# MoseleyBioinformaticsLab/pdb_eda

Measured on AMD Instinct MI355X. Metric: Mvoxels/s blob-labelled, higher is better.
Workload: dtype f32; 1 GPU; configs[1]: 256^3 synthetic CCP4 grid (gaussian-filtered noise, sigma_filter 1.5 voxels), fused green/red blob labelling at +-(mean+1.5*std), per-blob fp64 stats + dense int32 labels of both signs, map resident in HBM; labels=True, entries_per_rank=1

## Files before the change

### pdb_eda_amd/csrc/pdbeda_hip.hip

```cpp
#include <hip/hip_runtime.h>
#include <fcntl.h>
#include <sys/mman.h>
#include <sys/stat.h>
#include <unistd.h>
#include <cerrno>

#include <algorithm>
#include <chrono>
#include <thread>
#include <atomic>
#include <random>
#include <climits>
#include <cmath>
#include <cstdarg>
#include <cstdio>
#include <cstring>
#include <condition_variable>
#include <deque>
#include <map>
#include <mutex>
#include <string>
#include <vector>

#include "pdbeda_kernels.h"
// ... 1035 lines not shown
    pdbeda_ctx *ctx = m->ctx;
    HIP_TRY(ctx, hipSetDevice(ctx->device));
    return with_scratch(ctx, align_up(12 * n) + align_up(24 * n), [&](char *base) -> int {
        Carver cv(base);
        int32_t *d_crs = cv.take<int32_t>(3 * n);
        double *d_xyz = cv.take<double>(3 * n);
        const int32_t *in = pinned_in(ctx, crs, (size_t)(3 * n));
        if (!in) { HIP_TRY(ctx, h2d_one(ctx, d_crs, crs, (size_t)(12 * n))); in = d_crs; }
        double *res = pinned_out(ctx, xyz, (size_t)(3 * n));
        hipLaunchKernelGGL(k_crs2xyz, dim3(grid_for(n, 256)), dim3(256), 0, ctx->stream, m->geom_dev, in, n, res ? res : d_xyz);
        if (!res) HIP_TRY(ctx, d2h(ctx, xyz, d_xyz, 24 * n));
        return 0;
    });
}

extern "C" int pdbeda_xyz2crs(pdbeda_map *m, const double *xyz, int64_t n, int32_t *crs) {
    if (!m || (n > 0 && (!crs || !xyz)) || n < 0) return PDBEDA_ERR_ARGUMENT;
    if (n == 0) return PDBEDA_OK;
    pdbeda_ctx *ctx = m->ctx;
    HIP_TRY(ctx, hipSetDevice(ctx->device));
    return with_scratch(ctx, align_up(12 * n) + align_up(24 * n), [&](char *base) -> int {
        Carver cv(base);
        double *d_xyz = cv.take<double>(3 * n);
        int32_t *d_crs = cv.take<int32_t>(3 * n);
        const double *in = pinned_in(ctx, xyz, (size_t)(3 * n));
        if (!in) { HIP_TRY(ctx, h2d_one(ctx, d_xyz, xyz, (size_t)(24 * n))); in = d_xyz; }
        int32_t *res = pinned_out(ctx, crs, (size_t)(3 * n));
        hipLaunchKernelGGL(k_xyz2crs, dim3(grid_for(n, 256)), dim3(256), 0, ctx->stream, m->geom_dev, in, n, res ? res : d_crs);
        if (!res) HIP_TRY(ctx, d2h(ctx, crs, d_crs, 12 * n));
        return 0;
    });
}

static size_t job_carve(Job &job, char *base, int n_vols, int64_t total_words, int64_t total_keys, int64_t max_runs,
                        int64_t max_blobs, size_t extra_labels, int32_t **labels_out, int64_t n_tiles = 0, int64_t max_comps = -1) {
    if (max_comps < 0) max_comps = max_runs;
    job.run_cap = (uint32_t)max_runs; job.comp_cap = (uint32_t)max_comps; job.blob_cap = (uint32_t)std::min<int64_t>(max_blobs, 0xffffffffll);
    Carver cv(base);
    job.n_vols = n_vols;
    job.total_words = total_words;
    job.key_words = (total_keys + 63) / 64;
    job.n_fine = (int32_t)((job.key_words + KEY_FINE - 1) / KEY_FINE);
    job.fine_shift = 4;
    while (((int64_t)KEY_GROUPS << job.fine_shift) < job.n_fine) job.fine_shift++;
    job.fine_per_group = 1 << job.fine_shift;
    job.n_groups = (job.n_fine + job.fine_per_group - 1) / job.fine_per_group;
    job.vols = cv.take<VolDesc>(std::max(n_vols, 1));
    job.ctr = cv.take<Counters>(1);
    job.mask = cv.take<uint64_t>(total_words);
    job.key_bits = cv.take<uint64_t>((size_t)(job.key_words + KEY_FINE - 1) / KEY_FINE * KEY_FINE);
    job.n_fine_alloc = (int32_t)((job.n_fine + job.fine_per_group - 1) / job.fine_per_group * job.fine_per_group);
    job.fine_count = cv.take<uint32_t>((size_t)std::max(job.n_fine_alloc / 2, 8));
    job.mid_count = cv.take<uint32_t>((size_t)(job.key_words + KEY_FINE - 1) / KEY_FINE * (KEY_FINE / 16));
    job.group_count = (n_tiles && job.fine_shift > 4) ? cv.take<uint32_t>(KEY_GROUPS) : nullptr;
    job.run_base = cv.take<uint32_t>(total_words);
    job.comps_are_runs = n_tiles ? 0 : 1;
    job.comp_of_run = n_tiles ? cv.take<uint32_t>(max_runs) : nullptr;
    job.label_of_comp = n_tiles ? cv.take<int32_t>(max_comps) : nullptr;
    job.word_comps = n_tiles ? cv.take<uint8_t>((size_t)n_tiles * 2 * 256 * 8) : nullptr;
    job.unit_done = n_tiles ? cv.take<uint32_t>((size_t)n_tiles) : nullptr;
    job.unit_flag = n_tiles ? cv.take<uint32_t>(4) : nullptr;
    job.tile_mode = n_tiles ? cv.take<uint8_t>(n_tiles) : nullptr;
    job.tile_runs = n_tiles ? cv.take<uint32_t>(n_tiles) : nullptr;
    job.root_mask = n_tiles ? cv.take<uint64_t>((size_t)n_tiles * 4) : nullptr;
    job.n_tiles = (int32_t)n_tiles;
    if (n_tiles) {
        const int64_t nt = n_tiles, nfc = job.n_fine_alloc / 2, nmid = (job.key_words + KEY_FINE - 1) / KEY_FINE * (KEY_FINE / 16);
        job.clear_bits = (int32_t)((job.key_words + nt - 1) / nt);
        job.clear_fine = (int32_t)((nfc + nt - 1) / nt);
        job.clear_mid = (int32_t)((nmid + nt - 1) / nt);
    }
    job.inbox = n_tiles ? cv.take<InboxEntry>((size_t)n_tiles * INBOX_CAP) : nullptr;
    job.inbox_count = n_tiles ? cv.take<uint32_t>((size_t)n_tiles * INBOX_STRIDE) : nullptr;
    job.vol_sign[0] = job.vol_sign[1] = 1;
    job.parent = cv.take<int32_t>(max_comps);
    job.kpar = n_tiles ? cv.take<unsigned long long>(max_comps) : nullptr;
    job.r_n = cv.take<uint32_t>(max_comps);
    job.r_sum = cv.take<long long>((size_t)7 * max_comps);
    job.r_sum_stride = max_comps;
    job.r_c = cv.take<long long>(max_comps);
    job.r_r = cv.take<long long>(max_comps);
    job.r_s = cv.take<long long>(max_comps);
    job.r_key = cv.take<unsigned long long>(max_comps);
    job.r_rank = cv.take<uint32_t>(max_comps);
    job.b_n = cv.take<int64_t>(max_blobs);
    job.b_key = cv.take<int64_t>(max_blobs);
    job.b_total = cv.take<double>(max_blobs);
    job.b_centroid = cv.take<double>(3 * max_blobs);
    job.b_center = cv.take<double>(3 * max_blobs);
    job.b_volume = cv.take<double>(max_blobs);
    job.b_group = cv.take<int32_t>(max_blobs);
    int32_t *lab = extra_labels ? cv.take<int32_t>(extra_labels) : nullptr;
    if (labels_out) *labels_out = lab;
    return cv.off;
}

static int engine_enqueue(pdbeda_ctx *ctx, pdbeda_map *m, Job &job, int64_t max_runs, bool labelled = false, bool unordered = false) {
    hipStream_t st = ctx->stream;
    const unsigned run_grid = grid_for(max_runs, 256, 2048);
    if (job.total_words > 0 && !labelled) {
        {
            PROF(ctx, "k_run_index");
            static const int force_wpb = [] { const char *e = getenv("PDBEDA_RUNINDEX_WPB"); return e ? atoi(e) : 0; }();
            if (force_wpb != 256 && (force_wpb == 64 || (job.total_words < 256ll * 2048 && job.total_words > 64ll * job.n_vols))) hipLaunchKernelGGL(k_run_index<64>, dim3(grid_for(job.total_words, 64, 1ll << 30)), dim3(256), 0, st, job, m->dens, m->geom_dev);
            else hipLaunchKernelGGL(k_run_index<256>, dim3(grid_for(job.total_words, 256, 1ll << 30)), dim3(256), 0, st, job, m->dens, m->geom_dev);
        }
        { PROF(ctx, "k_union"); hipLaunchKernelGGL(k_union, dim3(grid_for(job.total_words * 4, 256, 1ll << 30)), dim3(256), 0, st, job); }
// ... 79 lines not shown
    const int64_t worst_unit = (int64_t)((uc + 1) / 2) * ur * us * n_planes + 1;
    if (tile_runs + worst_unit >= (1ll << 31))
        return fail(ctx, PDBEDA_ERR_ARGUMENT, "grid too large for whole-map labelling: %d x %d x %d voxels need %lld run ids (limit 2^31: about 1100^3 for a fused job)",
                    uc, ur, us, (long long)(tile_runs + worst_unit));
    const int64_t unit_ids = tier == 0 ? std::min<int64_t>(worst_unit, std::max<int64_t>(65536, tile_runs / 4)) : worst_unit;
    const int64_t max_blobs = tier == 0 ? std::min<int64_t>(worst_blobs, std::max<int64_t>(4096, total_keys / 32)) : worst_blobs;
    const int64_t max_runs = tile_runs + unit_ids, max_comps = tile_comps + unit_ids;

    int rc_fix = map_fix_mul(m);
    if (rc_fix) return rc_fix;
    Job job;
    memset(&job, 0, sizeof job);
    job.fix_mul = m->fix_mul;
    size_t need = job_carve(job, nullptr, n_planes, total_words, total_keys, max_runs, max_blobs, lab_elems, nullptr, tiles_pp, max_comps);
    Arena arena;
    int rc = arena_get(ctx, need, &arena);
    if (rc) return rc;
    int32_t *labels_dev = nullptr;
    job_carve(job, arena.base, n_planes, total_words, total_keys, max_runs, max_blobs, lab_elems, &labels_dev, tiles_pp, max_comps);
    job.vol_sign[0] = td.sign[0];
    job.vol_sign[1] = td.sign[1];
    job.unit_form = unit_form;
    static std::atomic<uint32_t> g_epoch{[] {
        uint32_t seed;
        try { seed = (uint32_t)std::random_device{}(); }
        catch (...) { seed = (uint32_t)std::chrono::steady_clock::now().time_since_epoch().count() ^ ((uint32_t)getpid() * 2654435761u); }
        return seed | 1u;
    }()};
    do { job.epoch = g_epoch.fetch_add(1u); } while (job.epoch == 0u || job.epoch == 0xffffffffu);

    JobInit init;
    memset(&init, 0, sizeof init);
    for (int p = 0; p < n_planes; ++p) {
        VolDesc &v = init.v[p];
        v.dim[0] = uc; v.dim[1] = ur; v.dim[2] = us;
        v.org[0] = v.org[1] = v.org[2] = 0;
        v.row_words = row_words;
        v.group = p;
        v.word_base = words_pp * p;
        v.key_base = keys_pp * p;
    }
    init.runs0 = (unsigned)tile_runs;
    init.comps0 = (unsigned)tile_comps;
    hipStream_t st = ctx->stream;
    int pair_slots = PAIR_SLOTS;
    if (ctx->debug_edge_cap > 0) { pair_slots = 1; while (pair_slots * 2 <= std::min<int64_t>(ctx->debug_edge_cap, PAIR_SLOTS)) pair_slots *= 2; }
    switch (td.cw) {
        case 1: launch_tile_label<1>(ctx, (unsigned)tiles_pp, job, m->dens, m->geom_dev, td, init, pair_slots); break;
        case 2: launch_tile_label<2>(ctx, (unsigned)tiles_pp, job, m->dens, m->geom_dev, td, init, pair_slots); break;
        case 3: launch_tile_label<3>(ctx, (unsigned)tiles_pp, job, m->dens, m->geom_dev, td, init, pair_slots); break;
        default: launch_tile_label<4>(ctx, (unsigned)tiles_pp, job, m->dens, m->geom_dev, td, init, pair_slots); break;
    }
    { PROF(ctx, "k_resolve_tiles"); hipLaunchKernelGGL(k_resolve_tiles, dim3((unsigned)tiles_pp + 64u), dim3(256), 0, st, job, (int)tiles_pp); }
    if (job.group_count) { PROF(ctx, "k_group_counts"); hipLaunchKernelGGL(k_group_counts, dim3((unsigned)(job.n_groups + 255) / 256u), dim3(256), 0, st, job); }
    if (labels) {
        PROF(ctx, "k_labels_tiles");
        launch_labels<true>(ctx, job, td, labels_dev, m->geom_dev);
    } else {
        PROF(ctx, "k_emit_tiles");
        hipLaunchKernelGGL(k_emit_tiles, dim3(std::min<unsigned>(512u, ((unsigned)tiles_pp + 1u) / 2u)), dim3(256), 0, st, job, m->geom_dev);
    }
    hipError_t e = hipGetLastError();
    if (e != hipSuccess) { arena_put(ctx, arena); return fail(ctx, PDBEDA_ERR_DEVICE, "whole-map labelling launch: %s", hipGetErrorString(e)); }
    out->job = job; out->arena = arena; out->td = td; out->labels_dev = labels_dev; out->labels = labels; out->bytes = need;
    return PDBEDA_OK;
}

static int full_blobs_impl(pdbeda_map *m, float cut_pos, float cut_neg, bool want_pos, bool want_neg, uint32_t flags,
                           pdbeda_bloblist **out_pos, pdbeda_bloblist **out_neg) {
    pdbeda_ctx *ctx = m->ctx;
    WholeMapJob wj;
    const int tier = ctx->debug_worst_case_arena ? 1 : 0, form = tier;
    int rc = whole_map_enqueue(m, cut_pos, cut_neg, want_pos, want_neg, flags, tier, form, &wj);
    if (rc) return rc;
    const int n_planes = (want_pos ? 1 : 0) + (want_neg ? 1 : 0);
    pdbeda_bloblist *first = nullptr;
    for (int p = 0; p < n_planes; ++p) {
        pdbeda_bloblist *bl = new_list(ctx, m);
        bl->job = wj.job;
        bl->td = wj.td;
        bl->vol_lo = p;
        bl->vol_hi = p + 1;
        bl->whole_map = true;
        bl->sign = wj.td.sign[p];
        if (p == 0) { bl->arena = wj.arena; bl->owns_arena = true; first = bl; }
        else { bl->owns_arena = false; bl->sibling = first; first->sibling = bl; }
        bl->labels_dev = wj.labels_dev;
        bl->labels_done = wj.labels;
        bl->cut_pos = cut_pos; bl->cut_neg = cut_neg; bl->want_pos = want_pos; bl->want_neg = want_neg; bl->flags = flags; bl->tier = tier; bl->unit_form = form;
        bl->job_bytes = wj.bytes;
        if (bl->sign > 0) *out_pos = bl; else *out_neg = bl;
    }
    return PDBEDA_OK;
}

extern "C" int pdbeda_full_blobs(pdbeda_map *m, float cutoff, uint32_t flags, pdbeda_bloblist **out) {
    if (!m || !out) return PDBEDA_ERR_ARGUMENT;
    *out = nullptr;
    if (cutoff == 0.0f || cutoff != cutoff) return fail(m->ctx, PDBEDA_ERR_ARGUMENT, "cutoff must be non-zero (the reference returns None)");
    pdbeda_bloblist *dummy = nullptr;
    if (cutoff > 0) return full_blobs_impl(m, cutoff, 0.0f, true, false, flags, out, &dummy);
    return full_blobs_impl(m, 0.0f, cutoff, false, true, flags, &dummy, out);
}

extern "C" int pdbeda_full_blobs_pm(pdbeda_map *m, float cutoff_pos, float cutoff_neg, uint32_t flags, pdbeda_bloblist **green,
                                    pdbeda_bloblist **red) {
    if (!m || !green || !red) return PDBEDA_ERR_ARGUMENT;
// ... 1779 lines not shown
```

### pdb_eda_amd/csrc/pdbeda_kernels.h

```cpp
#pragma once
#include "pdbeda_device.h"

namespace pdbeda {

struct VolDesc {
    int32_t dim[3];
    int32_t org[3];
    int32_t row_words;
    int32_t group;
    int64_t word_base;
    int64_t key_base;
};

struct FixSums {
    long long rho, c_lo, c_hi, r_lo, r_hi, s_lo, s_hi;
};
__device__ inline long long fix_of(double v, double mul) { return __double2ll_rn(v * mul); }
__device__ inline void fix_limbs(__int128 v, long long &lo, long long &hi) {
    lo = (long long)(unsigned long long)((unsigned __int128)v & 0xffffffffu);
    hi = (long long)(v >> 32);
}
__device__ inline double fix_moment(long long lo, long long hi) { return (double)hi * 4294967296.0 + (double)lo; }
__device__ inline FixSums fix_sums(long long F, long long m_c, long long m_r, long long m_s, long long c0, long long r0, long long s0) {
    FixSums o;
// ... 531 lines not shown
    unsigned long long c = 0, r = 0, sv = 0, key = ~0ull;
    if (root >= 0) {
        n = job.r_n[i]; sum = fix_load(job, i);
        c = (unsigned long long)job.r_c[i]; r = (unsigned long long)job.r_r[i]; sv = (unsigned long long)job.r_s[i]; key = job.r_key[i];
    }
    unsigned long long todo = __ballot(root >= 0);
    while (todo) {
        const int first = ctz64(todo);
        const int r0 = __shfl(root, first);
        const bool mine = root == r0;
        const unsigned long long group = __ballot(mine);
        todo &= ~group;
        uint32_t gn = mine ? n : 0u;
        FixSums g_sum = mine ? sum : fix_zero();
        unsigned long long g_c = mine ? c : 0ull, g_r = mine ? r : 0ull, g_s = mine ? sv : 0ull, g_key = mine ? key : ~0ull;
        if (group & (group - 1)) {
#pragma unroll
            for (int d = 32; d > 0; d >>= 1) {
                gn += __shfl_xor(gn, d);
                g_sum.rho += __shfl_xor(g_sum.rho, d);
                g_sum.c_lo += __shfl_xor(g_sum.c_lo, d); g_sum.c_hi += __shfl_xor(g_sum.c_hi, d);
                g_sum.r_lo += __shfl_xor(g_sum.r_lo, d); g_sum.r_hi += __shfl_xor(g_sum.r_hi, d);
                g_sum.s_lo += __shfl_xor(g_sum.s_lo, d); g_sum.s_hi += __shfl_xor(g_sum.s_hi, d);
                g_c += __shfl_xor(g_c, d); g_r += __shfl_xor(g_r, d); g_s += __shfl_xor(g_s, d);
                const unsigned long long k2 = __shfl_xor(g_key, d);
                g_key = k2 < g_key ? k2 : g_key;
            }
        }
        if (lane == first) {
            atomicAdd(&job.r_n[r0], gn);
            fix_fold(job, (uint32_t)r0, g_sum);
            atomicAdd((unsigned long long *)&job.r_c[r0], g_c);
            atomicAdd((unsigned long long *)&job.r_r[r0], g_r);
            atomicAdd((unsigned long long *)&job.r_s[r0], g_s);
            atomicMin(&job.r_key[r0], g_key);
        }
    }
}
__global__ void __launch_bounds__(256) k_resolve(Job job, int slots) {
    const uint32_t n_runs = n_components(job);
    const int lane = lane_id();
    const uint32_t stride = gridDim.x * blockDim.x;
    for (uint32_t i0 = blockIdx.x * blockDim.x + (threadIdx.x & ~63u); i0 < n_runs; i0 += stride)
        resolve_wave(job, i0 + (uint32_t)lane, i0 + (uint32_t)lane < n_runs, lane, slots != 0);
}

template <typename JobRef>
__device__ __forceinline__ void paint_key(const JobRef &job, unsigned long long key) {
    const uint32_t f = (uint32_t)((key >> 6) / KEY_FINE);
    const uint32_t cell = (uint32_t)(key >> 8);
    atomicOr((unsigned long long *)&job.key_bits[key >> 6], 1ull << (key & 63));
    atomicAdd(&job.mid_count[cell >> 2], 1u << ((cell & 3u) * 8u));
    atomicAdd(&job.fine_count[f >> 1], 1u << ((f & 1u) * 16u));
}

__global__ void __launch_bounds__(256) k_paint_keys(Job job) {
    const uint32_t n_runs = n_components(job);
    for (uint32_t i = blockIdx.x * blockDim.x + threadIdx.x; i < n_runs; i += gridDim.x * blockDim.x) {
        const int32_t par = job.parent[i];
        const uint32_t cnt = job.r_n[i];
        const unsigned long long key = job.r_key[i];
        if (par != (int32_t)i || cnt == 0u) continue;
        paint_key(job, key);
    }
}

template <int CTRL, int ROW_MASK = 0xf>
__device__ __forceinline__ uint32_t dpp0(uint32_t x) {
    return (uint32_t)__builtin_amdgcn_update_dpp(0, (int)x, CTRL, ROW_MASK, 0xf, true);
}
constexpr int DPP_ROW_SHR = 0x110, DPP_WAVE_SHR1 = 0x138, DPP_ROW_BCAST15 = 0x142, DPP_ROW_BCAST31 = 0x143;
__device__ __forceinline__ uint32_t half_scan(uint32_t x) {
    x += dpp0<DPP_ROW_SHR + 1>(x);
    x += dpp0<DPP_ROW_SHR + 2>(x);
    x += dpp0<DPP_ROW_SHR + 4>(x);
    x += dpp0<DPP_ROW_SHR + 8>(x);
    x += dpp0<DPP_ROW_BCAST15, 0xa>(x);
    return x;
}

__device__ __forceinline__ uint32_t wave_scan(uint32_t x) {
    x = half_scan(x);
    x += dpp0<DPP_ROW_BCAST31, 0xc>(x);
    return x;
}
__device__ __forceinline__ uint32_t sum_u16x8(const uint4 q) {
    const uint32_t a = (q.x & 0xffffu) + (q.x >> 16), b = (q.y & 0xffffu) + (q.y >> 16), c = (q.z & 0xffffu) + (q.z >> 16), d = (q.w & 0xffffu) + (q.w >> 16);
    return (a + b) + (c + d);
}
__device__ __forceinline__ uint32_t sum_u16_first(const uint4 q, int take) {
    const uint32_t w[4] = {q.x, q.y, q.z, q.w};
    uint32_t acc = 0;
#pragma unroll
    for (int k = 0; k < 4; ++k) acc += (2 * k < take ? (w[k] & 0xffffu) : 0u) + (2 * k + 1 < take ? (w[k] >> 16) : 0u);
    return acc;
}

template <int NT>
struct RankTableLoads {
    static constexpr int PER = KEY_GROUPS / NT;
    uint4 q[2 * PER];
    uint32_t v[PER];
    bool summed;
};
template <int NT = 256, typename JobRef = Job>
__device__ __forceinline__ void rank_table_issue(const JobRef &job, RankTableLoads<NT> &ld) {
    constexpr int PER = KEY_GROUPS / NT;
    const int tid = threadIdx.x;
    const int G = job.fine_per_group, n_groups = job.n_groups, Q = G / 8;
    const uint4 *fine4 = reinterpret_cast<const uint4 *>(job.fine_count);
    ld.summed = Q != 2;
    if (Q == 2) {
#pragma unroll
        for (int k = 0; k < PER; ++k) {
            const int e = tid * PER + k;
            ld.q[2 * k] = e < n_groups ? fine4[(size_t)e * 2] : make_uint4(0, 0, 0, 0);
            ld.q[2 * k + 1] = e < n_groups ? fine4[(size_t)e * 2 + 1] : make_uint4(0, 0, 0, 0);
        }
    } else if (job.group_count) {
        const uint32_t *gc = job.group_count;
#pragma unroll
        for (int k = 0; k < PER; ++k) {
            const int e = tid * PER + k;
            ld.v[k] = e < n_groups ? gc[e] : 0u;
        }
    } else {
#pragma unroll
        for (int k = 0; k < PER; ++k) {
            const int e = tid * PER + k;
            uint32_t acc = 0;
            if (e < n_groups)
                for (int j = 0; j < Q; ++j) acc += sum_u16x8(fine4[(size_t)e * Q + j]);
            ld.v[k] = acc;
        }
    }
}
template <int NT = 256>
__device__ __forceinline__ uint32_t rank_table_finish(RankTableLoads<NT> &ld, uint32_t *s_pre , uint32_t *s_wave ) {
    constexpr int PER = KEY_GROUPS / NT;
    const int tid = threadIdx.x, lane = tid & 63, wv = tid >> 6;
    if (!ld.summed) {
#pragma unroll
        for (int k = 0; k < PER; ++k) ld.v[k] = sum_u16x8(ld.q[2 * k]) + sum_u16x8(ld.q[2 * k + 1]);
    }
    uint32_t mine = 0;
#pragma unroll
    for (int k = 0; k < PER; ++k) mine += ld.v[k];
    const uint32_t x = wave_scan(mine);
    if (lane == 63) s_wave[wv] = x;
    __syncthreads();
    uint32_t pre = x - mine, total = 0;
#pragma unroll
    for (int k = 0; k < NT / 64; ++k) { const uint32_t w = s_wave[k]; pre += k < wv ? w : 0u; total += w; }
#pragma unroll
    for (int k = 0; k < PER; ++k) { s_pre[tid * PER + k] = pre; pre += ld.v[k]; }
    __syncthreads();
    return total;
}
template <int NT = 256, typename JobRef = Job>
__device__ inline uint32_t rank_table_lds(const JobRef &job, uint32_t *s_pre , uint32_t *s_wave ) {
    RankTableLoads<NT> ld;
    rank_table_issue<NT>(job, ld);
    return rank_table_finish<NT>(ld, s_pre, s_wave);
}

__global__ void __launch_bounds__(256) k_group_counts(Job job) {
    const int e = (int)(blockIdx.x * blockDim.x + threadIdx.x);
    if (e >= job.n_groups) return;
    const int Q = job.fine_per_group / 8;
    const uint4 *fine4 = reinterpret_cast<const uint4 *>(job.fine_count) + (size_t)e * Q;
    uint32_t acc = 0;
    for (int j = 0; j < Q; j += 4) {
        const uint4 a = fine4[j], b = fine4[j + 1], c = fine4[j + 2], d = fine4[j + 3];
        acc += (sum_u16x8(a) + sum_u16x8(b)) + (sum_u16x8(c) + sum_u16x8(d));
    }
    job.group_count[e] = acc;
}

struct RankLoads {
    uint4 q0, q1;
    uint2 mid;
    ulonglong2 b0, b1;
};
template <typename JobRef>
__device__ __forceinline__ void rank_issue(const JobRef &job, unsigned long long key, RankLoads &ld) {
    const uint32_t kw = (uint32_t)(key >> 6), f = kw / (uint32_t)KEY_FINE, e = f >> 4;
    const uint4 *fine4 = reinterpret_cast<const uint4 *>(job.fine_count) + (size_t)e * 2;
    ld.q0 = fine4[0]; ld.q1 = fine4[1];
    ld.mid = reinterpret_cast<const uint2 *>(job.mid_count)[f];
    const ulonglong2 *bits2 = reinterpret_cast<const ulonglong2 *>(job.key_bits + (kw & ~3u));
    ld.b0 = bits2[0]; ld.b1 = bits2[1];
}
__device__ __forceinline__ uint32_t rank_finish(const uint32_t *s_pre, unsigned long long key, const RankLoads &ld) {
    const uint32_t kw = (uint32_t)(key >> 6), f = kw / (uint32_t)KEY_FINE, e = f >> 4;
    const int nf = (int)(f & 15u), cell = (int)((kw & (uint32_t)(KEY_FINE - 1)) >> 2), wi = (int)(kw & 3u);
    uint32_t rank = s_pre[e] + sum_u16_first(ld.q0, nf) + sum_u16_first(ld.q1, nf - 8);
    const uint32_t lo = cell >= 4 ? ld.mid.x : (ld.mid.x & ((1u << (8 * cell)) - 1u));
    const uint32_t hi = cell > 4 ? (ld.mid.y & ((1u << (8 * (cell - 4))) - 1u)) : 0u;
    rank += __builtin_amdgcn_sad_u8(lo, 0u, 0u) + __builtin_amdgcn_sad_u8(hi, 0u, 0u);
    const uint64_t below = bits_below((int)(key & 63));
    const uint64_t w[4] = {ld.b0.x, ld.b0.y, ld.b1.x, ld.b1.y};
#pragma unroll
    for (int k = 0; k < 4; ++k) rank += (uint32_t)popc64(k < wi ? w[k] : (k == wi ? w[k] & below : 0ull));
    return rank;
}
template <typename JobRef>
__device__ inline uint32_t rank_of_key(const JobRef &job, const uint32_t *s_pre, unsigned long long key) {
    const int shift = job.fine_shift;
    if (shift == 4) {
        RankLoads ld;
        rank_issue(job, key, ld);
        return rank_finish(s_pre, key, ld);
    }
    const uint32_t kw = (uint32_t)(key >> 6), f = kw / (uint32_t)KEY_FINE, e = f >> shift;
    const int Q = 1 << (shift - 3);
    uint32_t rank = s_pre[e];
    const uint4 *fine4 = reinterpret_cast<const uint4 *>(job.fine_count) + (size_t)e * Q;
    const int nf = (int)(f - (e << shift));
    const uint2 mid = reinterpret_cast<const uint2 *>(job.mid_count)[f];
    const ulonglong2 *bits2 = reinterpret_cast<const ulonglong2 *>(job.key_bits + (kw & ~3u));
    const int cell = (int)((kw & (uint32_t)(KEY_FINE - 1)) >> 2);
    const int wi = (int)(kw & 3u);
    const ulonglong2 b0 = bits2[0], b1 = bits2[1];
    for (int k = 0; k * 8 < nf; ++k) rank += sum_u16_first(fine4[k], nf - k * 8);
    {
        const uint32_t lo = cell >= 4 ? mid.x : (mid.x & ((1u << (8 * cell)) - 1u));
        const uint32_t hi = cell > 4 ? (mid.y & ((1u << (8 * (cell - 4))) - 1u)) : 0u;
        rank += __builtin_amdgcn_sad_u8(lo, 0u, 0u) + __builtin_amdgcn_sad_u8(hi, 0u, 0u);
    }
    const uint64_t below = bits_below((int)(key & 63));
    const uint64_t w[4] = {b0.x, b0.y, b1.x, b1.y};
#pragma unroll
    for (int k = 0; k < 4; ++k) rank += (uint32_t)popc64(k < wi ? w[k] : (k == wi ? w[k] & below : 0ull));
    return rank;
}

__device__ __forceinline__ int nth_set_bit(uint64_t m, int k) {
    int pos = 0;
#pragma unroll
    for (int w = 32; w > 0; w >>= 1) {
        const int c = popc64(m & ((1ull << w) - 1ull));
        if (k >= c) { k -= c; m >>= w; pos += w; }
    }
    return pos;
}

template <typename JobRef>
__device__ __forceinline__ void emit_row_ranked(const JobRef &job, const Geom &g, bool whole_map, int64_t key_base1, uint32_t id, uint32_t n_vox,
                                                unsigned long long first_key, const FixSums &fs, long long ic, long long ir, long long is, uint32_t rank) {
    const double tot_q = (double)fs.rho, rc = fix_moment(fs.c_lo, fs.c_hi), rr = fix_moment(fs.r_lo, fs.r_hi), rs = fix_moment(fs.s_lo, fs.s_hi);
    const double tot = tot_q / job.fix_mul;
    const int vi = whole_map ? ((int64_t)first_key >= key_base1 ? 1 : 0) : find_vol_by_key(job.vols, job.n_vols, (int64_t)first_key);
    if (whole_map) job.label_of_comp[id] = job.vol_sign[vi] > 0 ? 1 + (int32_t)rank : -1 - (int32_t)rank;
    const VolDesc vd = job.vols[vi];
    job.r_rank[id] = rank;
    if (rank >= job.blob_cap) return;
    const double n = (double)n_vox;
    double wc[3] = {rc / tot_q, rr / tot_q, rs / tot_q};
    double cc[3] = {(double)ic / n, (double)ir / n, (double)is / n};
    double xyz[3];
    crs2xyz_frac(g, wc, xyz);
    job.b_centroid[3 * rank + 0] = xyz[0];
    job.b_centroid[3 * rank + 1] = xyz[1];
    job.b_centroid[3 * rank + 2] = xyz[2];
    crs2xyz_frac(g, cc, xyz);
    job.b_center[3 * rank + 0] = xyz[0];
    job.b_center[3 * rank + 1] = xyz[1];
    job.b_center[3 * rank + 2] = xyz[2];
    job.b_n[rank] = (int64_t)n_vox;
    job.b_total[rank] = tot;
    job.b_volume[rank] = g.unit_volume * n;
    job.b_key[rank] = (int64_t)first_key - vd.key_base;
    job.b_group[rank] = vd.group;
}
template <typename JobRef>
__device__ __forceinline__ void emit_row(const JobRef &job, const Geom &g, const uint32_t *s_pre, bool whole_map, int64_t key_base1, uint32_t id,
                                         uint32_t n_vox, unsigned long long first_key, const FixSums &fs, long long ic, long long ir, long long is) {
    emit_row_ranked(job, g, whole_map, key_base1, id, n_vox, first_key, fs, ic, ir, is, rank_of_key(job, s_pre, first_key));
}

template <typename JobRef>
__device__ inline void emit_ids(const JobRef &job, const Geom &g, const uint32_t *s_pre, bool whole_map, int64_t key_base1, uint32_t first, uint32_t n_comp,
                                uint32_t block, uint32_t n_blocks) {
    const uint32_t stride = n_blocks * blockDim.x;
    uint32_t i = first + block * blockDim.x + threadIdx.x;
    int32_t par = i < n_comp ? job.parent[i] : -1;
    uint32_t cnt = i < n_comp ? job.r_n[i] : 0u;
    unsigned long long key = i < n_comp ? job.r_key[i] : 0ull;
    for (; i < n_comp; i += stride) {
        const bool root = par == (int32_t)i && cnt != 0u;
        const uint32_t nx = i + stride;
        const int32_t par_next = nx < n_comp ? job.parent[nx] : -1;
        const uint32_t cnt_next = nx < n_comp ? job.r_n[nx] : 0u;
        const unsigned long long key_next = nx < n_comp ? job.r_key[nx] : 0ull;
        if (root) emit_row(job, g, s_pre, whole_map, key_base1, i, cnt, key, fix_load(job, i), job.r_c[i], job.r_r[i], job.r_s[i]);
        par = par_next;
        cnt = cnt_next;
        key = key_next;
    }
}

__global__ void __launch_bounds__(256) k_emit(Job job, const Geom *__restrict__ gp) {
    __shared__ uint32_t s_pre[KEY_GROUPS];
    __shared__ uint32_t s_wave[4];
    const uint32_t total = rank_table_lds(job, s_pre, s_wave);
    emit_ids(job, *gp, s_pre, false, INT64_MAX, 0u, n_components(job), blockIdx.x, gridDim.x);
    if (blockIdx.x == 0 && threadIdx.x == 0) {
        job.ctr->n_blobs = total;
        job.ctr->n_blobs_vol0 = total;
        if (total > job.blob_cap) atomicOr(&job.ctr->overflow, 2u);
    }
}

__global__ void __launch_bounds__(256) k_emit_tiles(Job job, const Geom *__restrict__ gp) {
    __shared__ uint32_t s_pre[KEY_GROUPS];
    __shared__ uint32_t s_wave[4];
    __shared__ unsigned long long s_acc[2][10][TILE_COMPS];
    __shared__ uint32_t s_accn[2][TILE_COMPS];
    const int half = threadIdx.x >> 7, k0 = threadIdx.x & 127;
    const int n_tiles = job.n_tiles;
    int tile = (int)blockIdx.x * 2 + half;
    uint64_t rm[4] = {0ull, 0ull, 0ull, 0ull};
    uint32_t n_in = 0;
    if (tile < n_tiles) {
#pragma unroll
        for (int q = 0; q < 4; ++q) rm[q] = job.root_mask[(size_t)tile * 4 + q];
        n_in = job.inbox_count[(size_t)tile * INBOX_STRIDE];
    }
    const int64_t key_base1 = job.n_vols > 1 ? job.vols[1].key_base : INT64_MAX;
    const uint32_t total = rank_table_lds(job, s_pre, s_wave);
    const Geom &g = *gp;
    for (int t0 = (int)blockIdx.x * 2; t0 < n_tiles; t0 += (int)gridDim.x * 2) {
        tile = t0 + half;
        n_in = min(n_in, (uint32_t)INBOX_CAP);
        const int next = tile + (int)gridDim.x * 2;
        uint64_t nm[4] = {0ull, 0ull, 0ull, 0ull};
        uint32_t n_in_next = 0;
        if (next < n_tiles) {
#pragma unroll
            for (int q = 0; q < 4; ++q) nm[q] = job.root_mask[(size_t)next * 4 + q];
            n_in_next = job.inbox_count[(size_t)next * INBOX_STRIDE];
        }
        InboxEntry e0, e1;
        const bool have0 = (uint32_t)k0 < n_in, have1 = (uint32_t)k0 + 128u < n_in;
        if (have0) e0 = job.inbox[(size_t)tile * INBOX_CAP + k0];
        if (have1) e1 = job.inbox[(size_t)tile * INBOX_CAP + k0 + 128];
        if (n_in != 0u) {
#pragma unroll
            for (int f = 0; f < 10; ++f) { s_acc[half][f][k0] = 0ull; s_acc[half][f][k0 + 128] = 0ull; }
            s_accn[half][k0] = 0u; s_accn[half][k0 + 128] = 0u;
        }
        __syncthreads();
        auto absorb = [&](const InboxEntry &e) {
            const uint32_t l = e.local;
            atomicAdd(&s_accn[half][l], e.n);
            atomicAdd(&s_acc[half][0][l], (unsigned long long)e.sum.rho);
            atomicAdd(&s_acc[half][1][l], (unsigned long long)e.sum.c_lo); atomicAdd(&s_acc[half][2][l], (unsigned long long)e.sum.c_hi);
            atomicAdd(&s_acc[half][3][l], (unsigned long long)e.sum.r_lo); atomicAdd(&s_acc[half][4][l], (unsigned long long)e.sum.r_hi);
            atomicAdd(&s_acc[half][5][l], (unsigned long long)e.sum.s_lo); atomicAdd(&s_acc[half][6][l], (unsigned long long)e.sum.s_hi);
            atomicAdd(&s_acc[half][7][l], e.c); atomicAdd(&s_acc[half][8][l], e.r); atomicAdd(&s_acc[half][9][l], e.s);
        };
        if (have0) absorb(e0);
        if (have1) absorb(e1);
        __syncthreads();
        const int c0 = popc64(rm[0]), c1 = c0 + popc64(rm[1]), c2 = c1 + popc64(rm[2]), n_roots = c2 + popc64(rm[3]);
        for (int k = k0; k < n_roots; k += 128) {
            const int q = k < c0 ? 0 : (k < c1 ? 1 : (k < c2 ? 2 : 3));
            const int before = q == 0 ? 0 : (q == 1 ? c0 : (q == 2 ? c1 : c2));
            const uint64_t word = q == 0 ? rm[0] : (q == 1 ? rm[1] : (q == 2 ? rm[2] : rm[3]));
            const uint32_t l = (uint32_t)(64 * q + nth_set_bit(word, k - before));
            const uint32_t id = (uint32_t)tile * (uint32_t)TILE_COMPS + l;
            uint32_t n_vox = job.r_n[id];
            const unsigned long long key = job.r_key[id];
            FixSums fs = fix_load(job, id);
            long long ic = job.r_c[id], ir = job.r_r[id], is = job.r_s[id];
            if (n_in != 0u) {
                n_vox += s_accn[half][l];
                fs.rho += (long long)s_acc[half][0][l];
                fs.c_lo += (long long)s_acc[half][1][l]; fs.c_hi += (long long)s_acc[half][2][l];
                fs.r_lo += (long long)s_acc[half][3][l]; fs.r_hi += (long long)s_acc[half][4][l];
                fs.s_lo += (long long)s_acc[half][5][l]; fs.s_hi += (long long)s_acc[half][6][l];
                ic += (long long)s_acc[half][7][l]; ir += (long long)s_acc[half][8][l]; is += (long long)s_acc[half][9][l];
            }
// ... 1281 lines not shown
```

### pdb_eda_amd/csrc/pdbeda_tile.h

```cpp
#pragma once
#include "pdbeda_kernels.h"
#include <type_traits>

namespace pdbeda {

constexpr int TILE_R = 8, TILE_S = 8;
constexpr int RCAP = 1408;
constexpr int RCAP_DENSE = 4096;
constexpr int CCAP = 256;
static_assert(CCAP == TILE_COMPS, "k_emit walks the tiles' component ranges");
constexpr int VCAP = 3584;
constexpr int FACE_K = 7;

struct TileDims {
    int cw;
    int ctiles, rtiles, stiles;
    int n_planes;
    int uc, ur, us, row_words;
    int nc, nr;
    float cut[2];
    int sign[2];
};

__host__ __device__ inline int64_t tile_index(const TileDims &td, int plane, int wq, int r, int s) {
// ... 632 lines not shown
    const unsigned long long *comps64 = reinterpret_cast<const unsigned long long *>(lj.word_comps);
    auto word_at = [&](int q, int r, int s, int wq) { return (int64_t)q * plane_words + ((int64_t)s * ur + r) * row_words + wq; };
    auto comps_at = [&](uint32_t tl, int q, int r, int s, int wl) { return ((size_t)tl * 2 + q) * 256 + ((s & 7) * TILE_R + (r & 7)) * CW + wl; };
    auto comp_by_run = [&](int64_t w, uint32_t k) { return lj.comp_of_run[lj.run_base[w] + k]; };

    const int fq = tid / (FACE_PAIRS * 4), frem = tid % (FACE_PAIRS * 4), ft = frem >> 2, fwl = frem & 3;
    int rl = 0, sl = 0, dr = 0, ds = -1;
    bool task = tid < 2 * FACE_PAIRS * 4 && fq < td.n_planes && fwl < CW && w0 + fwl < row_words;
    if (ft < 8) { rl = 0; sl = ft; dr = -1; ds = 0; }
    else if (ft < 16) { rl = 0; sl = ft - 8; dr = -1; }
    else if (ft < 23) { rl = ft - 15; sl = 0; dr = -1; }
    else if (ft < 31) { rl = ft - 23; sl = 0; dr = 0; }
    else if (ft < 39) { rl = ft - 31; sl = 0; dr = 1; }
    else { rl = 7; sl = ft - 38; dr = 1; }
    const int r = rt * TILE_R + rl, s = st * TILE_S + sl, r2 = r + dr, s2 = s + ds;
    if (r >= ur || s >= us || r2 < 0 || r2 >= ur || s2 < 0) task = false;
    const uint32_t tile_b = task ? (uint32_t)(((s2 >> 3) * td.rtiles + (r2 >> 3)) * td.ctiles + ct) : 0u;
    const int64_t wA = task ? word_at(fq, r, s, w0 + fwl) : 0, wB = task ? word_at(fq, r2, s2, w0 + fwl) : 0;
    uint64_t mA = 0ull, mB = 0ull;
    unsigned long long cA = 0ull, cB = 0ull;
    uint32_t modes = 0u;
    if (task) {
        mA = lj.mask[wA]; mB = lj.mask[wB];
        cA = comps64[comps_at((uint32_t)tile, fq, r, s, fwl)]; cB = comps64[comps_at(tile_b, fq, r2, s2, fwl)];
        modes = (uint32_t)lj.tile_mode[tile] | (uint32_t)lj.tile_mode[tile_b];
    }
    uint32_t tiles5[5];
    {
        const int drs[5] = {0, -1, -1, 0, 1}, dss[5] = {0, 0, -1, -1, -1};
#pragma unroll
        for (int j = 0; j < 5; ++j) {
            const int r5 = rt + drs[j], s5 = st + dss[j];
            tiles5[j] = (r5 >= 0 && r5 < td.rtiles && s5 >= 0) ? (uint32_t)((s5 * td.rtiles + r5) * td.ctiles + ct) : 0xffffffffu;
        }
    }
    constexpr int KPL = (5 * KPH + NTH - 1) / NTH;
    kp_t kp_pre[KPL];
#pragma unroll
    for (int k = 0; k < KPL; ++k) {
        const int e = tid + k * NTH, j = e / KPH;
        const uint32_t t5 = j == 0 ? tiles5[0] : (j == 1 ? tiles5[1] : (j == 2 ? tiles5[2] : (j == 3 ? tiles5[3] : tiles5[4])));
        kp_pre[k] = (e < 5 * KPH && t5 != 0xffffffffu) ? kuf_load(lj.kpar, t5 * (uint32_t)CCAP + (uint32_t)(e % KPH)) : KP_UNUSED;
    }
    {
        const int64_t key_words = lj.key_words;
        const int64_t lo = (int64_t)lj.clear_bits * tile, hi = lo + lj.clear_bits < key_words ? lo + lj.clear_bits : key_words;
        for (int64_t i = lo + tid; i < hi; i += NTH) lj.key_bits[i] = 0ull;
        const int64_t nfc = lj.n_fine_alloc / 2;
        const int64_t clo = (int64_t)lj.clear_fine * tile, chi = clo + lj.clear_fine < nfc ? clo + lj.clear_fine : nfc;
        for (int64_t i = clo + tid; i < chi; i += NTH) lj.fine_count[i] = 0u;
        const int64_t nmid = (key_words + KEY_FINE - 1) / KEY_FINE * (KEY_FINE / 16);
        const int64_t mlo = (int64_t)lj.clear_mid * tile, mhi = mlo + lj.clear_mid < nmid ? mlo + lj.clear_mid : nmid;
        for (int64_t i = mlo + tid; i < mhi; i += NTH) lj.mid_count[i] = 0u;
        if (tid == 0) lj.inbox_count[(size_t)tile * INBOX_STRIDE] = 0u;
    }
    for (int i = tid; i < pair_slots; i += NTH) s_set[i] = 0ull;
#pragma unroll
    for (int k = 0; k < KPL; ++k) {
        const int e = tid + k * NTH;
        if (e < 5 * KPH) (&s_kp[0][0])[e] = kp_pre[k];
    }
    lds_barrier();
    auto val_of = [&](uint32_t id) -> kp_t {
        const uint32_t t = id / (uint32_t)CCAP;
#pragma unroll
        for (int j = 0; j < 5; ++j)
            if (t == tiles5[j] && (id % (uint32_t)CCAP) < (uint32_t)KPH) return s_kp[j][id % (uint32_t)CCAP];
        return kuf_load(lj.kpar, id);
    };
    const uint32_t slot_mask = (uint32_t)pair_slots - 1u;
    auto add_pair = [&](uint32_t ca, uint32_t cb) {
        const uint32_t lo = ca < cb ? ca : cb, hi = ca < cb ? cb : ca;
        const unsigned long long key = ((unsigned long long)lo << 32) | hi;
        uint32_t h = (uint32_t)((key * 0x9E3779B97F4A7C15ull) >> 40) & slot_mask;
        for (int probe = 0; probe < 8; ++probe, h = (h + 1u) & slot_mask) {
            const unsigned long long old = atomicCAS(&s_set[h], 0ull, key);
            if (old == 0ull || old == key) return;
        }
        kuf_hook_vals(lj.kpar, val_of(lo), val_of(hi));
    };
    {
        if (modes != 0u) { mA = 0ull; mB = 0ull; }
        const uint64_t SA = mA & ~(mA << 1), SB = mB & ~(mB << 1);
        const uint32_t pack = (uint32_t)(mA >> 63) | ((uint32_t)(mB >> 63) << 1) | ((uint32_t)(cA >> 56) << 8) | ((uint32_t)(cB >> 56) << 16);
        uint32_t prev = dpp0<DPP_WAVE_SHR1>(pack);
        if (fwl == 0) prev = 0u;
        const uint64_t carA = prev & 1u, carB = (prev >> 1) & 1u;
        uint64_t todo = (SA & (mB | (mB << 1) | carB)) | (SB & ((mA << 1) | carA));
        const uint32_t baseA = (uint32_t)tile * CCAP, baseB = tile_b * CCAP;
        uint32_t last_a = ~0u, last_b = ~0u;
        while (todo) {
            const int p = ctz64(todo);
            todo &= todo - 1ull;
            const uint64_t upto = (2ull << p) - 1ull;
            const uint32_t ka = (uint32_t)popc64(SA & upto), kb = (uint32_t)popc64(SB & upto);
            uint32_t ca, cb;
            if (ka == 0u) ca = baseA + ((prev >> 8) & 0xffu);
            else ca = ka <= (uint32_t)FACE_K ? baseA + (uint32_t)((cA >> ((ka - 1u) * 8u)) & 0xffull) : comp_by_run(wA, ka - 1u);
            if (kb == 0u) cb = baseB + ((prev >> 16) & 0xffu);
            else cb = kb <= (uint32_t)FACE_K ? baseB + (uint32_t)((cB >> ((kb - 1u) * 8u)) & 0xffull) : comp_by_run(wB, kb - 1u);
            if (ca != last_a || cb != last_b) {
                add_pair(ca, cb);
                last_a = ca; last_b = cb;
            }
        }
    }
// ... 197 lines not shown
        } else {
            fold(root, s_cnt[k], s_f[k], s_i[0][k], s_i[1][k], s_i[2][k]);
        }
    }
}

constexpr int LCAP = 4096;
#ifndef PDBEDA_LABELS_NT_THREADS
#define PDBEDA_LABELS_NT_THREADS 512
#endif
template <int CW, bool FUSED>
__global__ void __launch_bounds__(PDBEDA_LABELS_NT_THREADS, FUSED ? 8 : 1) k_labels_tiles(Job job_arg, TileDims td, int32_t *__restrict__ labels, const Geom *__restrict__ gp) {
    kernarg_prefetch();
    PDBEDA_LATE_JOB(lj);
    constexpr int NU = 64 * CW;
    constexpr int NTL = PDBEDA_LABELS_NT_THREADS, RPW = 64 / (NTL / 64);
    __shared__ int32_t s_lab[CCAP];
    __shared__ __attribute__((aligned(16))) uint2 s_mh[2 * 256];
    __shared__ __attribute__((aligned(16))) uint2 s_sb[2][2 * 256];
    __shared__ __attribute__((aligned(16))) unsigned char s_pc[(LCAP + 8) > 4 * KEY_GROUPS ? (LCAP + 8) : 4 * KEY_GROUPS];
    uint8_t *s_comp8 = s_pc;
    uint32_t *s_pre = reinterpret_cast<uint32_t *>(s_pc);
    __shared__ unsigned long long s_acc[FUSED ? 10 : 1][FUSED ? CCAP : 1];
    __shared__ uint32_t s_accn[FUSED ? CCAP : 1];
    __shared__ uint32_t s_wave[NTL / 64];
    __shared__ uint32_t s_vol0;
    const int tid = threadIdx.x, lane = tid & 63, wv = tid >> 6;
    const int wvs = __builtin_amdgcn_readfirstlane(wv);
    const int uc = td.uc, ur = td.ur, us = td.us, row_words = td.row_words;
    const int ct = (int)blockIdx.x, rt = (int)blockIdx.y, st = (int)blockIdx.z;
    const uint32_t bid = ((uint32_t)st * (uint32_t)td.rtiles + (uint32_t)rt) * (uint32_t)td.ctiles + (uint32_t)ct;
    const int w0 = ct * CW, r0 = rt * TILE_R, s0 = st * TILE_S;
    const int64_t plane_words = (int64_t)row_words * ur * us;
    const uint32_t rb = (uint32_t)bid * (uint32_t)(NU * 32), cb = (uint32_t)bid * CCAP;
    static_assert(NTL == 512 && LCAP == 4096, "two unconditional comp loads per thread cover the first 1024 runs");
    constexpr int CPRE = 2;
    uint32_t c_pre[CPRE];
#pragma unroll
    for (int k = 0; k < CPRE; ++k) c_pre[k] = lj.comp_of_run[rb + tid + NTL * k];
    const uint32_t c_pack = ((c_pre[0] - cb) & 0xffu) | (((c_pre[1] - cb) & 0xffu) << 8);
    int32_t lab_pre = 0;
    int32_t vol0 = 0;
    if (!FUSED) {
        lab_pre = tid < CCAP ? lj.label_of_comp[lj.parent[cb + tid]] : 0;
        vol0 = lj.n_vols > 1 ? (int32_t)lj.ctr->n_blobs_vol0 : 0;
    }
    kp_t kp = KP_UNUSED;
    const int64_t key_base1 = (FUSED && td.n_planes > 1) ? (int64_t)uc * ur * us : INT64_MAX;
    uint32_t n_in = 0;
    const uint32_t jd = cb + (uint32_t)(tid & 255);
    uint32_t rec_n = 0;
    FixSums rec_f = fix_zero();
    long long rec_c = 0, rec_r = 0, rec_s = 0;
    if (FUSED) {
        kp = kuf_load(lj.kpar, jd);
        n_in = lj.inbox_count[(size_t)bid * INBOX_STRIDE];
    }
    auto own_list = [&](int32_t lab) { return lab < 0 ? lab + vol0 : lab; };
    const bool unit = lj.tile_mode[(int64_t)bid] != 0;
    const uint32_t n_runs_raw = lj.tile_runs[bid];
    const uint32_t n_runs = unit ? 0u : n_runs_raw;
    const bool fast = !unit && n_runs <= (uint32_t)LCAP;
    const int pwl = tid % CW, prowl = (tid / CW) & 63;
    const int pr = r0 + (prowl & 7), ps = s0 + (prowl >> 3);
    const bool pvalid = tid < NU && pr < ur && ps < us && w0 + pwl < row_words;
    const int64_t pw = ((int64_t)ps * ur + pr) * row_words + (w0 + pwl);
    uint64_t m[2] = {0ull, 0ull};
    uint32_t base[2] = {0u, 0u};
    if (tid < 256) {
#pragma unroll
        for (int p = 0; p < 2; ++p) {
            const bool has = pvalid && p < td.n_planes;
            m[p] = has ? lj.mask[pw + p * plane_words] : 0ull;
            base[p] = has ? lj.run_base[pw + p * plane_words] : 0u;
        }
    }
    uint32_t total_blobs = 0, blobs_vol0 = 0;
    bool my_root = false;
    auto write_mask_tables = [&]() {
        if (tid < 256) {
            s_mh[2 * tid] = make_uint2((uint32_t)m[0], (uint32_t)m[1]);
            s_mh[2 * tid + 1] = make_uint2((uint32_t)(m[0] >> 32), (uint32_t)(m[1] >> 32));
#pragma unroll
            for (int p = 0; p < 2; ++p) {
                const uint64_t starts = run_starts(m[p]);
                const uint32_t slo = (uint32_t)starts, shi = (uint32_t)(starts >> 32), before = base[p] - rb - 1u;
                s_sb[p][2 * tid] = make_uint2(slo, before);
                s_sb[p][2 * tid + 1] = make_uint2(shi, before + (uint32_t)__popc(slo));
            }
        }
    };
    auto label_of_value = [&](kp_t v) -> int32_t {
        const uint32_t key32 = (uint32_t)(v >> 32);
        const int plane = (int)(key32 >> 31);
        const unsigned long long key = (unsigned long long)(plane ? key_base1 : 0) + (key32 & 0x7fffffffu);
        const int32_t rank = (int32_t)rank_of_key(lj, s_pre, key);
        return lj.vol_sign[plane] > 0 ? 1 + rank : -1 - rank;
    };
    if (FUSED) {
        static_assert(10 * CCAP == 5 * NTL, "five accumulator words per thread");
#pragma unroll
        for (int k = 0; k < 5; ++k) (&s_acc[0][0])[tid + NTL * k] = 0ull;
        if (tid < CCAP) s_accn[tid] = 0u;
        total_blobs = rank_table_lds<NTL>(lj, s_pre, s_wave);
        n_in = min(n_in, (uint32_t)INBOX_CAP);
        write_mask_tables();
        static_assert(INBOX_CAP <= 256, "an inbox entry per thread of the lower half");
        const bool used = kp != KP_UNUSED;
        static_assert(sizeof(InboxEntry) == 88, "eleven words");
        const bool have = (uint32_t)(tid & 255) < n_in;
        const unsigned long long *ew = reinterpret_cast<const unsigned long long *>(lj.inbox + (size_t)bid * INBOX_CAP + (tid & 255));
        my_root = tid >= 256 && used && kp_id(kp) == jd;
        if (tid < 256) {
            unsigned long long e_head = 0ull, e_w[4] = {0ull, 0ull, 0ull, 0ull};
            if (have) {
                e_head = ew[0];
#pragma unroll
                for (int k = 0; k < 4; ++k) e_w[k] = ew[1 + k];
            }
            const bool vol0_lane = tid == 255 && key_base1 != INT64_MAX;
            int32_t raw = 0;
            if (used || vol0_lane) {
                const uint32_t key32 = (uint32_t)(kp >> 32);
                const int plane = used ? (int)(key32 >> 31) : 1;
                const unsigned long long key = (unsigned long long)(plane ? key_base1 : 0) + (used ? (key32 & 0x7fffffffu) : 0u);
                const int32_t rank = (int32_t)rank_of_key(lj, s_pre, key);
                if (used) raw = lj.vol_sign[plane] > 0 ? 1 + rank : -1 - rank;
                else s_vol0 = (uint32_t)rank;
            }
            if (vol0_lane && used) s_vol0 = rank_of_key(lj, s_pre, (unsigned long long)key_base1);
            if (tid == 255 && key_base1 == INT64_MAX) s_vol0 = total_blobs;
            s_lab[tid] = raw;
            if (have) {
                const uint32_t l = (uint32_t)e_head;
                atomicAdd(&s_accn[l], (uint32_t)(e_head >> 32));
#pragma unroll
                for (int k = 0; k < 4; ++k) atomicAdd(&s_acc[k][l], e_w[k]);
            }
        } else {
            unsigned long long e_head = 0ull, e_w[6] = {0ull, 0ull, 0ull, 0ull, 0ull, 0ull};
            if (have) {
                e_head = ew[0];
#pragma unroll
                for (int k = 0; k < 6; ++k) e_w[k] = ew[5 + k];
            }
            if (my_root) {
                rec_n = lj.r_n[jd];
                rec_f = fix_load(lj, jd);
                rec_c = lj.r_c[jd]; rec_r = lj.r_r[jd]; rec_s = lj.r_s[jd];
            }
            if (have) {
                const uint32_t l = (uint32_t)e_head;
#pragma unroll
                for (int k = 0; k < 6; ++k) atomicAdd(&s_acc[4 + k][l], e_w[k]);
            }
        }
        __syncthreads();
// ... 51 lines not shown
            const unsigned snib = (sb.x >> sh) & 0xfu;
            const unsigned upto_first = (2u << __builtin_ctz(nib)) - 1u;
            const uint32_t run = sb.y + (uint32_t)__popc(sb.x & lowm) + (uint32_t)__popc(snib & upto_first);
            const unsigned s2 = snib & ~upto_first;
            const unsigned from2 = 0u - (s2 & (0u - s2));
            const unsigned abits = nib & ~from2, bbits = nib & from2;
            int32_t la, lb;
            if (FAST) { la = s_lab[s_comp8[run]]; lb = s_lab[s_comp8[run + 1u]]; }
            else {
                la = label_of_run(run + rb);
                lb = s2 ? label_of_run(run + rb + 1u) : 0;
            }
#pragma unroll
            for (int k = 0; k < 4; ++k)
                o[k] |= (__builtin_amdgcn_sbfe((int)abits, k, 1) & la) | (__builtin_amdgcn_sbfe((int)bbits, k, 1) & lb);
        };
        constexpr int ROW_UNROLL = FAST ? RPW : 1;
#pragma unroll ROW_UNROLL
        for (int rr = 0; rr < RPW; ++rr) {
            const int rowl = wvs * RPW + rr;
            const int r = r0 + (rowl & 7), s = s0 + (rowl >> 3);
            if (!INSIDE && (r >= ur || s >= us)) continue;
            if (hsel >= 2 * CW || (!INSIDE && c >= uc)) continue;
            const int hidx = rowl * (2 * CW) + hsel;
            const uint2 mh = s_mh[hidx];
            const unsigned nib0 = (mh.x >> sh) & 0xfu, nib1 = (mh.y >> sh) & 0xfu;
            int32_t out[4] = {0, 0, 0, 0};
            {
                const bool second = nib0 == 0u;
                const unsigned nib = second ? nib1 : nib0;
                if (nib) group(second ? 1 : 0, nib, hidx, out);
            }
            if (__ballot(nib0 != 0u && nib1 != 0u)) {
                if (nib0 != 0u && nib1 != 0u) group(1, nib1, hidx, out);
            }
            int32_t *dst = labels + ((int64_t)s * ur + r) * uc + c;
            if (INSIDE || (c + 3 < uc && ((uc & 3) == 0))) {
                typedef int v4i __attribute__((ext_vector_type(4)));
                const v4i o4 = {out[0], out[1], out[2], out[3]};
                __builtin_nontemporal_store(o4, reinterpret_cast<v4i *>(dst));
            } else {
#pragma unroll
                for (int q = 0; q < 4; ++q)
                    if (c + q < uc) dst[q] = out[q];
            }
        }
    };
    if (fast) { if (inside) rows(std::true_type{}, std::true_type{}); else rows(std::true_type{}, std::false_type{}); }
    else { if (inside) rows(std::false_type{}, std::true_type{}); else rows(std::false_type{}, std::false_type{}); }
    if (FUSED) {
        const bool any_unit = *lj.unit_flag == lj.epoch;
        if (any_unit) {
            __syncthreads();
            rank_table_lds<NTL>(lj, s_pre, s_wave);
            const uint32_t n_comp = n_components(lj), first = (uint32_t)lj.n_tiles * (uint32_t)TILE_COMPS;
            if (n_comp > first && lj.ctr->overflow == 0u) emit_ids(lj, *gp, s_pre, true, key_base1, first, n_comp, bid, (uint32_t)lj.n_tiles);
        }
    }
}

__global__ void k_labels_decode(const int32_t *__restrict__ signed_labels, int64_t n, int sign, int32_t *__restrict__ out) {
    for (int64_t i = (int64_t)blockIdx.x * blockDim.x + threadIdx.x; i < n; i += (int64_t)gridDim.x * blockDim.x) {
        const int32_t v = signed_labels[i];
        out[i] = sign > 0 ? (v > 0 ? v - 1 : -1) : (v < 0 ? -v - 1 : -1);
    }
}

}
```

Before: 227,900 Mvoxels/s.

## Maintain per-group key counts atomically during key painting, drop group-count kernel

Key painting now also bumps a per-group counter with one atomic per key, and the group counters are zeroed inside the tile-label kernel's clear phase. This removes the separate k_group_counts launch. The rank-table build in the resolve and label kernels then reads one vector of group totals per thread instead of summing packed fine counts. The label kernel also issues the rank-table loads early so their latency overlaps the other setup work. The cost is an extra global atomic per painted key, which may contend on hot groups.

```diff
diff --git a/pdb_eda_amd/csrc/pdbeda_hip.hip b/pdb_eda_amd/csrc/pdbeda_hip.hip
--- a/pdb_eda_amd/csrc/pdbeda_hip.hip
+++ b/pdb_eda_amd/csrc/pdbeda_hip.hip
@@ -1111,7 +1111,7 @@
     job.n_fine_alloc = (int32_t)((job.n_fine + job.fine_per_group - 1) / job.fine_per_group * job.fine_per_group);
     job.fine_count = cv.take<uint32_t>((size_t)std::max(job.n_fine_alloc / 2, 8));
     job.mid_count = cv.take<uint32_t>((size_t)(job.key_words + KEY_FINE - 1) / KEY_FINE * (KEY_FINE / 16));
-    job.group_count = (n_tiles && job.fine_shift > 4) ? cv.take<uint32_t>(KEY_GROUPS) : nullptr;
+    job.group_count = n_tiles ? cv.take<uint32_t>(KEY_GROUPS) : nullptr;
     job.run_base = cv.take<uint32_t>(total_words);
     job.comps_are_runs = n_tiles ? 0 : 1;
     job.comp_of_run = n_tiles ? cv.take<uint32_t>(max_runs) : nullptr;
@@ -1297,7 +1297,6 @@
         default: launch_tile_label<4>(ctx, (unsigned)tiles_pp, job, m->dens, m->geom_dev, td, init, pair_slots); break;
     }
     { PROF(ctx, "k_resolve_tiles"); hipLaunchKernelGGL(k_resolve_tiles, dim3((unsigned)tiles_pp + 64u), dim3(256), 0, st, job, (int)tiles_pp); }
-    if (job.group_count) { PROF(ctx, "k_group_counts"); hipLaunchKernelGGL(k_group_counts, dim3((unsigned)(job.n_groups + 255) / 256u), dim3(256), 0, st, job); }
     if (labels) {
         PROF(ctx, "k_labels_tiles");
         launch_labels<true>(ctx, job, td, labels_dev, m->geom_dev);
diff --git a/pdb_eda_amd/csrc/pdbeda_kernels.h b/pdb_eda_amd/csrc/pdbeda_kernels.h
--- a/pdb_eda_amd/csrc/pdbeda_kernels.h
+++ b/pdb_eda_amd/csrc/pdbeda_kernels.h
@@ -607,6 +607,8 @@
     atomicOr((unsigned long long *)&job.key_bits[key >> 6], 1ull << (key & 63));
     atomicAdd(&job.mid_count[cell >> 2], 1u << ((cell & 3u) * 8u));
     atomicAdd(&job.fine_count[f >> 1], 1u << ((f & 1u) * 16u));
+    uint32_t *gc = job.group_count;
+    if (gc) atomicAdd(&gc[f >> job.fine_shift], 1u);
 }
 
 __global__ void __launch_bounds__(256) k_paint_keys(Job job) {
@@ -651,17 +653,25 @@
     return acc;
 }
 
-template <int NT>
+template <int NT, bool TOTALS = false>
 struct RankTableLoads {
     static constexpr int PER = KEY_GROUPS / NT;
-    uint4 q[2 * PER];
+    uint4 q[TOTALS ? 1 : 2 * PER];
     uint32_t v[PER];
     bool summed;
 };
-template <int NT = 256, typename JobRef = Job>
-__device__ __forceinline__ void rank_table_issue(const JobRef &job, RankTableLoads<NT> &ld) {
+template <int NT = 256, bool TOTALS = false, typename JobRef = Job>
+__device__ __forceinline__ void rank_table_issue(const JobRef &job, RankTableLoads<NT, TOTALS> &ld) {
     constexpr int PER = KEY_GROUPS / NT;
     const int tid = threadIdx.x;
+    if (TOTALS) {
+        typedef uint32_t vec_t __attribute__((ext_vector_type(PER)));
+        const vec_t t = reinterpret_cast<const vec_t *>(job.group_count)[tid];
+#pragma unroll
+        for (int k = 0; k < PER; ++k) ld.v[k] = t[k];
+        ld.summed = true;
+        return;
+    }
     const int G = job.fine_per_group, n_groups = job.n_groups, Q = G / 8;
     const uint4 *fine4 = reinterpret_cast<const uint4 *>(job.fine_count);
     ld.summed = Q != 2;
@@ -671,13 +681,6 @@
             const int e = tid * PER + k;
             ld.q[2 * k] = e < n_groups ? fine4[(size_t)e * 2] : make_uint4(0, 0, 0, 0);
             ld.q[2 * k + 1] = e < n_groups ? fine4[(size_t)e * 2 + 1] : make_uint4(0, 0, 0, 0);
-        }
-    } else if (job.group_count) {
-        const uint32_t *gc = job.group_count;
-#pragma unroll
-        for (int k = 0; k < PER; ++k) {
-            const int e = tid * PER + k;
-            ld.v[k] = e < n_groups ? gc[e] : 0u;
         }
     } else {
 #pragma unroll
@@ -690,11 +693,11 @@
         }
     }
 }
-template <int NT = 256>
-__device__ __forceinline__ uint32_t rank_table_finish(RankTableLoads<NT> &ld, uint32_t *s_pre , uint32_t *s_wave ) {
+template <int NT = 256, bool TOTALS = false>
+__device__ __forceinline__ uint32_t rank_table_finish(RankTableLoads<NT, TOTALS> &ld, uint32_t *s_pre , uint32_t *s_wave ) {
     constexpr int PER = KEY_GROUPS / NT;
     const int tid = threadIdx.x, lane = tid & 63, wv = tid >> 6;
-    if (!ld.summed) {
+    if (!TOTALS && !ld.summed) {
 #pragma unroll
         for (int k = 0; k < PER; ++k) ld.v[k] = sum_u16x8(ld.q[2 * k]) + sum_u16x8(ld.q[2 * k + 1]);
     }
@@ -712,24 +715,11 @@
     __syncthreads();
     return total;
 }
-template <int NT = 256, typename JobRef = Job>
+template <int NT = 256, bool TOTALS = false, typename JobRef = Job>
 __device__ inline uint32_t rank_table_lds(const JobRef &job, uint32_t *s_pre , uint32_t *s_wave ) {
-    RankTableLoads<NT> ld;
-    rank_table_issue<NT>(job, ld);
-    return rank_table_finish<NT>(ld, s_pre, s_wave);
-}
-
-__global__ void __launch_bounds__(256) k_group_counts(Job job) {
-    const int e = (int)(blockIdx.x * blockDim.x + threadIdx.x);
-    if (e >= job.n_groups) return;
-    const int Q = job.fine_per_group / 8;
-    const uint4 *fine4 = reinterpret_cast<const uint4 *>(job.fine_count) + (size_t)e * Q;
-    uint32_t acc = 0;
-    for (int j = 0; j < Q; j += 4) {
-        const uint4 a = fine4[j], b = fine4[j + 1], c = fine4[j + 2], d = fine4[j + 3];
-        acc += (sum_u16x8(a) + sum_u16x8(b)) + (sum_u16x8(c) + sum_u16x8(d));
-    }
-    job.group_count[e] = acc;
+    RankTableLoads<NT, TOTALS> ld;
+    rank_table_issue<NT, TOTALS>(job, ld);
+    return rank_table_finish<NT, TOTALS>(ld, s_pre, s_wave);
 }
 
 struct RankLoads {
@@ -760,13 +750,8 @@
     return rank;
 }
 template <typename JobRef>
-__device__ inline uint32_t rank_of_key(const JobRef &job, const uint32_t *s_pre, unsigned long long key) {
+__device__ inline uint32_t rank_of_key_wide(const JobRef &job, const uint32_t *s_pre, unsigned long long key) {
     const int shift = job.fine_shift;
-    if (shift == 4) {
-        RankLoads ld;
-        rank_issue(job, key, ld);
-        return rank_finish(s_pre, key, ld);
-    }
     const uint32_t kw = (uint32_t)(key >> 6), f = kw / (uint32_t)KEY_FINE, e = f >> shift;
     const int Q = 1 << (shift - 3);
     uint32_t rank = s_pre[e];
@@ -788,6 +773,15 @@
 #pragma unroll
     for (int k = 0; k < 4; ++k) rank += (uint32_t)popc64(k < wi ? w[k] : (k == wi ? w[k] & below : 0ull));
     return rank;
+}
+template <typename JobRef>
+__device__ inline uint32_t rank_of_key(const JobRef &job, const uint32_t *s_pre, unsigned long long key) {
+    if (job.fine_shift == 4) {
+        RankLoads ld;
+        rank_issue(job, key, ld);
+        return rank_finish(s_pre, key, ld);
+    }
+    return rank_of_key_wide(job, s_pre, key);
 }
 
 __device__ __forceinline__ int nth_set_bit(uint64_t m, int k) {
@@ -883,7 +877,7 @@
         n_in = job.inbox_count[(size_t)tile * INBOX_STRIDE];
     }
     const int64_t key_base1 = job.n_vols > 1 ? job.vols[1].key_base : INT64_MAX;
-    const uint32_t total = rank_table_lds(job, s_pre, s_wave);
+    const uint32_t total = rank_table_lds<256, true>(job, s_pre, s_wave);
     const Geom &g = *gp;
     for (int t0 = (int)blockIdx.x * 2; t0 < n_tiles; t0 += (int)gridDim.x * 2) {
         tile = t0 + half;
diff --git a/pdb_eda_amd/csrc/pdbeda_tile.h b/pdb_eda_amd/csrc/pdbeda_tile.h
--- a/pdb_eda_amd/csrc/pdbeda_tile.h
+++ b/pdb_eda_amd/csrc/pdbeda_tile.h
@@ -708,6 +708,7 @@
         const int64_t nmid = (key_words + KEY_FINE - 1) / KEY_FINE * (KEY_FINE / 16);
         const int64_t mlo = (int64_t)lj.clear_mid * tile, mhi = mlo + lj.clear_mid < nmid ? mlo + lj.clear_mid : nmid;
         for (int64_t i = mlo + tid; i < mhi; i += NTH) lj.mid_count[i] = 0u;
+        for (int64_t i = (int64_t)tile + (int64_t)tid * lj.n_tiles; i < KEY_GROUPS; i += (int64_t)NTH * lj.n_tiles) lj.group_count[i] = 0u;
         if (tid == 0) lj.inbox_count[(size_t)tile * INBOX_STRIDE] = 0u;
     }
     for (int i = tid; i < pair_slots; i += NTH) s_set[i] = 0ull;
@@ -1011,9 +1012,11 @@
     uint32_t rec_n = 0;
     FixSums rec_f = fix_zero();
     long long rec_c = 0, rec_r = 0, rec_s = 0;
+    RankTableLoads<NTL, true> tl;
     if (FUSED) {
         kp = kuf_load(lj.kpar, jd);
         n_in = lj.inbox_count[(size_t)bid * INBOX_STRIDE];
+        rank_table_issue<NTL, true>(lj, tl);
     }
     auto own_list = [&](int32_t lab) { return lab < 0 ? lab + vol0 : lab; };
     const bool unit = lj.tile_mode[(int64_t)bid] != 0;
@@ -1061,7 +1064,7 @@
 #pragma unroll
         for (int k = 0; k < 5; ++k) (&s_acc[0][0])[tid + NTL * k] = 0ull;
         if (tid < CCAP) s_accn[tid] = 0u;
-        total_blobs = rank_table_lds<NTL>(lj, s_pre, s_wave);
+        total_blobs = rank_table_finish<NTL, true>(tl, s_pre, s_wave);
         n_in = min(n_in, (uint32_t)INBOX_CAP);
         write_mask_tables();
         static_assert(INBOX_CAP <= 256, "an inbox entry per thread of the lower half");
@@ -1219,7 +1222,7 @@
         const bool any_unit = *lj.unit_flag == lj.epoch;
         if (any_unit) {
             __syncthreads();
-            rank_table_lds<NTL>(lj, s_pre, s_wave);
+            rank_table_lds<NTL, true>(lj, s_pre, s_wave);
             const uint32_t n_comp = n_components(lj), first = (uint32_t)lj.n_tiles * (uint32_t)TILE_COMPS;
             if (n_comp > first && lj.ctr->overflow == 0u) emit_ids(lj, *gp, s_pre, true, key_base1, first, n_comp, bid, (uint32_t)lj.n_tiles);
         }
```

New measurement: 208,000 Mvoxels/s. 0.913x the previous value.
